# facebookresearch/seamless_communication

Hardware: AMD Instinct MI355X
Metric: S2ST utterances/sec (and real-time factor), seamlessM4T_v2_large, 10 s audio (higher is better)
Workload: dtype f32 activations x f16 weights, f32 accumulate

## Files before the change

### seamless_communication_amd/csrc/common.cpp

```cpp
#include "common.h"
#include <cstdlib>
#include <cstring>

namespace sc {

static thread_local char g_err[1024] = "";

void set_error(const char* fmt, ...) {
    va_list ap;
    va_start(ap, fmt);
    vsnprintf(g_err, sizeof(g_err), fmt, ap);
    va_end(ap);
}

const char* get_error() { return g_err; }

namespace knob {
namespace {
struct Knob {
    const char* name;
    int kind;
    const char* what;
};
const Knob knob_table[] = {
// ... 4 lines not shown
    {"SC_DECODER_GEN2", 1, "decoder step on the second-generation chain"},
    {"SC_VOC_SPLIT", 1, "vocoder ResBlock products on both fp16 planes of their activations again (bit 0 wide stages, bit 2 narrow stages); default: hi plane only"},
    {"SC_GEMM_GENERAL", 0, "general GEMM kernel instead of the fast path"}, {"SC_GEMM_PF2", 0, "GEMM prefetch depth"},
    {"SC_GEMM_GROUP_M", 0, "GEMM workgroup order"}, {"SC_GEMM_TILE", 0, "GEMM tile override"},
    {"SC_PS_TILE", 0, "DMA GEMM: largest tile"}, {"SC_PS_MIN256", 0, "DMA GEMM: tiles needed for 256 x 256"},
    {"SC_PS_MIN128", 0, "DMA GEMM: tiles needed for 128 x 128"},
    {"SC_PRESPLIT", 0, "0: Conformer operands split on the fly"}, {"SC_ENC_FUSE", 0, "0: separate Conformer element-wise launches"},
    {"SC_D3_RG_SMALL", 0, "decoder step: rows per row group, N = 1024 products"}, {"SC_D3_RG_FFN", 0, "decoder step: rows per row group, FFN-in"},
    {"SC_G3_STATIONARY", 0, "row-group products of wide steps: 0 one workgroup per row group, n = workgroup budget of the weight-stationary launch"},
    {"SC_G3_TILES", 0, "0: FFN-out of wide steps on the weight-stationary row-group walk instead of tile-owning waves"},
    {"SC_G3_TOUCH", 0, "weight-stationary products: bit 0 cooperative L2 touch of the activations, bit 1 K slices per XCD (FFN-out); default 3"},
    {"SC_D3_FFN_IN", 0, "decoder step: FFN-in workgroup shape"}, {"SC_D3_FFN_OUT", 0, "decoder step: FFN-out workgroup shape"},
    {"SC_T2U_GROUPS", 0, "NAR T2U: length buckets"}, {"SC_T2U_PACKED", 0, "0: NAR decoder on padded buckets"},
    {"SC_VOC_PS", 0, "0: vocoder wide stages on the register-staged convolution"}, {"SC_VOC_MRF", 0, "0: narrow vocoder stages as nine pair launches"},
    {"SC_VOC_GROUPS", 0, "vocoder: length buckets"}, {"SC_VOC_GROUP_OVERHEAD", 0, "vocoder: bucket planning overhead rows"},
    {"SC_VOC_STREAMS", 0, "vocoder: side chains"},
    {"SC_VOC_PACKED", 0, "0: ragged vocoder batches in length buckets on side chains instead of the packed pass"},
    {"SC_VOC_PACK_ROWS", 0, "vocoder: unit rows per packed group"},
    {"SC_ENGINE_RG_SMALL", 0, "decode engine: rows per row group, N = 1024 products"},
    {"SC_BEAM_COMPACT", 2, "0: beam search keeps finished utterances' slots"},
    {"SC_GREEDY_COMPACT", 2, "0: greedy generation keeps finished rows in their slots"}, {"SC_GREEDY_POLL", 2, "steps between looks at the finished flags"},
    {"SC_T2U_ENC_PACKED", 2, "0: T2U encoder over the padded rows on the fp32-operand GEMM"},
    {"SC_ENC_GLU_EPI", 2, "0: Conformer conv module writes both GLU halves and gates them in the depthwise kernel"},
};
constexpr int N_KNOBS = sizeof(knob_table) / sizeof(knob_table[0]);
struct State {
    bool set[N_KNOBS];
    int val[N_KNOBS];
    bool numerics = false;
};
const State& state() {
    static const State st = [] {
        State s{};
        const char* dn = getenv("SC_DEBUG_NUMERICS");
        s.numerics = dn && atoi(dn) != 0;
        for (int i = 0; i < N_KNOBS; ++i) {
            const char* e = getenv(knob_table[i].name);
            s.set[i] = e != nullptr && (knob_table[i].kind != 1 || s.numerics);
            s.val[i] = e ? atoi(e) : 0;
        }
        return s;
    }();
    return st;
}
int lookup(const char* name) {
    for (int i = 0; i < N_KNOBS; ++i)
// ... 43 lines not shown
```

### seamless_communication_amd/csrc/k_gemm.hip

```cpp
#include <atomic>
#include <cstdlib>

#include "device_util.h"

namespace sc {

std::atomic<int> g_force_general_gemm{0};

static constexpr int BK = 32;
static constexpr int LDS_LD = 40;

__device__ __forceinline__ float apply_in_act(float v, int in_act) {
    if (in_act == IN_LRELU_01) return v > 0.f ? v : 0.1f * v;
    if (in_act == IN_LRELU_001) return v > 0.f ? v : 0.01f * v;
    return v;
}

template <int BM, int BN, int WGM, int WGN, int AMODE, bool SPLIT>
__global__ __launch_bounds__(256) void gemm_kernel(GemmArgs p) {
    static_assert(WGM * WGN == 4, "4 waves per block");
    constexpr int WM = BM / WGM, WN = BN / WGN;
    constexpr int TM = WM / 32, TN = WN / 32;
    static_assert(TM >= 1 && TN >= 1, "wave tile must hold a 32x32 fragment");
    constexpr int A_IT = BM / 32;
    constexpr int B_IT = (BN * 4 + 255) / 256;

    __shared__ __attribute__((aligned(16))) _Float16 sAh[BM * LDS_LD];
    __shared__ __attribute__((aligned(16))) _Float16 sAl[SPLIT ? BM * LDS_LD : 8];
    __shared__ __attribute__((aligned(16))) _Float16 sB[BN * LDS_LD];

    const int tid = threadIdx.x;
    const int lane = tid & 63;
    const int wave = tid >> 6;
    const int wm = wave / WGN, wn = wave % WGN;
    const int m0 = blockIdx.y * BM;
    const int n0 = blockIdx.x * BN;
    const int phase = blockIdx.z;
    const __half* __restrict__ W = p.W + (int64_t)phase * p.w_phase_stride;
    const int out_off = p.out_off + phase * p.out_off_phase_step;

    const int a_kq = tid & 7;
// ... 131 lines not shown
#pragma unroll
            for (int i = 0; i < TM; ++i) {
                const int off = (wm * WM + i * 32 + frag_row) * LDS_LD + kb + frag_k;
                ah[i] = *reinterpret_cast<const half8_t*>(&sAh[off]);
                if (SPLIT) al[i] = *reinterpret_cast<const half8_t*>(&sAl[off]);
            }
#pragma unroll
            for (int j = 0; j < TN; ++j) {
                const int off = (wn * WN + j * 32 + frag_row) * LDS_LD + kb + frag_k;
                bf[j] = *reinterpret_cast<const half8_t*>(&sB[off]);
            }
#pragma unroll
            for (int i = 0; i < TM; ++i)
#pragma unroll
                for (int j = 0; j < TN; ++j) {
                    acc[i][j] = __builtin_amdgcn_mfma_f32_32x32x16_f16(ah[i], bf[j], acc[i][j], 0, 0, 0);
                    if (SPLIT)
                        acc[i][j] = __builtin_amdgcn_mfma_f32_32x32x16_f16(al[i], bf[j], acc[i][j], 0, 0, 0);
                }
        }
        __syncthreads();
    }

    const bool plain_rows = !p.item_off && (p.rows_per_batch == p.M) && p.out_mul == 1 && out_off == 0 && p.t_out == p.M;
    if (p.item_off && m0 + wm * WM + 4 * (lane >> 5) < p.M) cur.init(p, m0 + wm * WM + 4 * (lane >> 5));
#pragma unroll
    for (int i = 0; i < TM; ++i) {
#pragma unroll
        for (int r = 0; r < 16; ++r) {
            const int m = m0 + wm * WM + i * 32 + (r & 3) + 8 * (r >> 2) + 4 * (lane >> 5);
            if (m >= p.M) continue;
            int64_t row;
            if (plain_rows) {
                row = m;
            } else if (p.item_off) {
                cur.seek(p, m);
                const int dst_t = cur.q(m) * p.out_mul + out_off;
                if (dst_t < 0 || dst_t >= cur.t_out(p)) continue;
                row = cur.out_row0(p) + dst_t;
            } else {
                const int n = m / p.rows_per_batch;
                const int q = m - n * p.rows_per_batch;
                const int dst_t = q * p.out_mul + out_off;
                if (dst_t < 0 || dst_t >= p.t_out) continue;
                row = (int64_t)n * p.t_out + dst_t;
            }
#pragma unroll
            for (int j = 0; j < TN; ++j) {
                const int col = n0 + wn * WN + j * 32 + (lane & 31);
                if (col >= p.N) continue;
                float v = acc[i][j][r];
                if (p.bias) v += p.bias[col];
                v = act(v, p.act) * p.alpha;
                if (p.res) v += p.res[row * p.ldr + col];
                p.C[row * p.ldc + col] = v;
            }
        }
    }
}

template <int BM, int BN, int WGM, int WGN>
static void launch_cfg(const GemmArgs& a, hipStream_t s) {
    dim3 grid(cdiv(a.N, BN), cdiv(a.M, BM), a.phases);
    const bool vec_ok = (a.lda % 4 == 0) && ((reinterpret_cast<uintptr_t>(a.A) & 15) == 0);
    const int amode = (vec_ok && a.cin % 32 == 0) ? 1 : (vec_ok && a.cin % 4 == 0) ? 2 : 0;
    char name[64];
    snprintf(name, sizeof(name), "gemm_%dx%d_%s_%s", BM, BN, amode == 1 ? "vecA" : amode == 2 ? "vec4A" : "genA",
             a.split ? "split" : "f16");
    const double kreal = (double)a.taps * a.cin;
    const double flops = a.algo_flops > 0 ? a.algo_flops : 2.0 * a.M * a.N * kreal * a.phases;
    const double bytes = 4.0 * a.M * (double)a.cin * (a.stride < a.taps ? 1.0 : (double)a.taps) +
                         2.0 * a.N * (double)a.K * a.phases + 4.0 * a.M * (double)a.N * (a.res ? 2.0 : 1.0);
    prof::Scope scope(name, flops, bytes, s);
#define SC_GEMM_LAUNCH(AM, SP) hipLaunchKernelGGL((gemm_kernel<BM, BN, WGM, WGN, AM, SP>), grid, dim3(256), 0, s, a)
    if (a.split) {
        if (amode == 1) SC_GEMM_LAUNCH(1, true);
        else if (amode == 2) SC_GEMM_LAUNCH(2, true);
        else SC_GEMM_LAUNCH(0, true);
    } else {
        if (amode == 1) SC_GEMM_LAUNCH(1, false);
        else if (amode == 2) SC_GEMM_LAUNCH(2, false);
        else SC_GEMM_LAUNCH(0, false);
    }
#undef SC_GEMM_LAUNCH
}

void launch_gemm(const GemmArgs& a, hipStream_t s) {
    SC_CHECK(a.K % BK == 0, "gemm: K=%d must be a multiple of %d", a.K, BK);
    SC_CHECK(a.ldw % 8 == 0, "gemm: ldw=%lld must be a multiple of 8", (long long)a.ldw);
    SC_CHECK(a.M > 0 && a.N > 0, "gemm: empty problem M=%d N=%d", a.M, a.N);
    SC_CHECK(a.rows_per_batch > 0 && a.cin > 0, "gemm: rows_per_batch/cin unset");
    static const bool env_general = knob::is_set("SC_GEMM_GENERAL");
    SC_CHECK(a.act >= ACT_NONE && a.act <= ACT_GELU, "gemm: unknown activation %d", a.act);
    if (!env_general && !g_force_general_gemm.load(std::memory_order_relaxed) && gemm_fast_eligible(a)) {
        launch_gemm_fast(a, s);
        return;
    }
    const int64_t tiles128 = (int64_t)cdiv(a.M, 128) * cdiv(a.N, 128) * a.phases;
    if (a.M <= 32) {
        launch_cfg<32, 128, 1, 4>(a, s);
    } else if (a.N <= 32) {
        if ((int64_t)cdiv(a.M, 256) * a.phases >= 512) launch_cfg<256, 32, 4, 1>(a, s);
        else launch_cfg<128, 32, 4, 1>(a, s);
    } else if (a.N <= 64) {
        if ((int64_t)cdiv(a.M, 128) * a.phases >= 512) launch_cfg<128, 64, 2, 2>(a, s);
        else launch_cfg<64, 64, 2, 2>(a, s);
    } else if (tiles128 >= 256) {
        launch_cfg<128, 128, 2, 2>(a, s);
    } else {
        launch_cfg<64, 64, 2, 2>(a, s);
    }
    SC_LAUNCH_CHECK();
}

template <int MR>
__global__ __launch_bounds__(256) void gemv_kernel(const float* __restrict__ x, int64_t ldx,
// ... 76 lines not shown
```

### seamless_communication_amd/csrc/k_gemm2.hip

```cpp
#include <algorithm>
#include <cstdlib>

#include "device_util.h"

namespace sc {

namespace {

constexpr int GEMM_GROUP_M_DEFAULT = 1;
constexpr int GEMM_PF2_DEFAULT = 1;
constexpr int FBK = 32;
constexpr int FLD = 40;

template <int TM, int TN, int WM, int WN, int ACT, bool HAS_RES>
__device__ __forceinline__ void epilogue(const GemmArgs& p, float16_t (&acc)[TM][TN], int m0w, int n0w, int lane,
                                         int out_off, bool plain_rows) {
    float bcol[TN];
    int col[TN];
#pragma unroll
    for (int j = 0; j < TN; ++j) {
        col[j] = n0w + j * 32 + (lane & 31);
        bcol[j] = (p.bias && col[j] < p.N) ? p.bias[col[j]] : 0.f;
    }
    GemmItemCursor cur;
    if (p.item_off && m0w + 4 * (lane >> 5) < p.M) cur.init(p, m0w + 4 * (lane >> 5));
#pragma unroll
    for (int i = 0; i < TM; ++i) {
#pragma unroll
        for (int r = 0; r < 16; ++r) {
            const int m = m0w + i * 32 + (r & 3) + 8 * (r >> 2) + 4 * (lane >> 5);
            if (m >= p.M) continue;
            int64_t row;
            if (plain_rows) {
                row = m;
            } else if (p.item_off) {
                cur.seek(p, m);
                const int dst_t = cur.q(m) * p.out_mul + out_off;
                if (dst_t < 0 || dst_t >= cur.t_out(p)) continue;
                row = cur.out_row0(p) + dst_t;
            } else {
                const int n = m / p.rows_per_batch;
                const int q = m - n * p.rows_per_batch;
                const int dst_t = q * p.out_mul + out_off;
                if (dst_t < 0 || dst_t >= p.t_out) continue;
                row = (int64_t)n * p.t_out + dst_t;
            }
#pragma unroll
            for (int j = 0; j < TN; ++j) {
                if (col[j] >= p.N) continue;
                float v = act<ACT>(acc[i][j][r] + bcol[j]) * p.alpha;
                if (HAS_RES) v += p.res[row * p.ldr + col[j]];
                p.C[row * p.ldc + col[j]] = v;
            }
        }
    }
}

template <int TM, int TN, int WN, int EP_LD, int ACT, bool HAS_RES>
__device__ __forceinline__ void epilogue_lds(const GemmArgs& p, float16_t (&acc)[TM][TN], float* ep, int m0w, int n0w, int lane,
                                             int out_off, bool plain_rows) {
    constexpr int LPR = WN / 4;
    constexpr int RPG = 16 / LPR;
    constexpr int RPI = 4 * RPG;
    const int l5 = lane & 31;
    const bool g1 = (l5 >= 4 && l5 < 12) || (l5 >= 16 && l5 < 20) || l5 >= 28;
    const int rank = g1 ? (l5 < 12 ? l5 - 4 : l5 < 20 ? l5 - 8 : l5 - 16) : (l5 < 4 ? l5 : l5 < 16 ? l5 - 8 : l5 - 12);
    const int grp = (lane >> 5) * 2 + (g1 ? 1 : 0);
    const int row_in = grp * RPG + rank / LPR;
    const int c0 = (rank % LPR) * 4;
    const int col = n0w + c0;
    const bool vec_ok = (col + 3 < p.N) && (p.ldc % 4 == 0) && (!HAS_RES || p.ldr % 4 == 0) &&
                        ((reinterpret_cast<uintptr_t>(p.C) | (HAS_RES ? reinterpret_cast<uintptr_t>(p.res) : 0)) & 15) == 0;
    f32x4_t b4 = {0.f, 0.f, 0.f, 0.f};
    if (p.bias) {
#pragma unroll
        for (int e = 0; e < 4; ++e) b4[e] = (col + e < p.N) ? p.bias[col + e] : 0.f;
    }
    GemmItemCursor cur;
    if (p.item_off && m0w + row_in < p.M) cur.init(p, m0w + row_in);
#pragma unroll
    for (int i = 0; i < TM; ++i) {
#pragma unroll
        for (int j = 0; j < TN; ++j)
#pragma unroll
            for (int r = 0; r < 16; ++r) ep[((r & 3) + 8 * (r >> 2) + 4 * (lane >> 5)) * EP_LD + j * 32 + (lane & 31)] = acc[i][j][r];
#pragma unroll
        for (int it = 0; it < 32 / RPI; ++it) {
            const int rr = it * RPI + row_in;
            const int m = m0w + i * 32 + rr;
            const f32x4_t a = *reinterpret_cast<const f32x4_t*>(ep + rr * EP_LD + c0);
            if (m >= p.M || col >= p.N) continue;
            int64_t row;
            if (plain_rows) {
                row = m;
            } else if (p.item_off) {
                cur.seek(p, m);
                const int dst_t = cur.q(m) * p.out_mul + out_off;
                if (dst_t < 0 || dst_t >= cur.t_out(p)) continue;
                row = cur.out_row0(p) + dst_t;
            } else {
                const int n = m / p.rows_per_batch;
                const int q = m - n * p.rows_per_batch;
                const int dst_t = q * p.out_mul + out_off;
                if (dst_t < 0 || dst_t >= p.t_out) continue;
                row = (int64_t)n * p.t_out + dst_t;
            }
            f32x4_t v;
#pragma unroll
            for (int e = 0; e < 4; ++e) v[e] = act<ACT>(a[e] + b4[e]) * p.alpha;
            if (vec_ok) {
                if (HAS_RES) v += *reinterpret_cast<const f32x4_t*>(p.res + row * p.ldr + col);
                *reinterpret_cast<f32x4_t*>(p.C + row * p.ldc + col) = v;
            } else {
#pragma unroll
                for (int e = 0; e < 4; ++e) {
                    if (col + e >= p.N) continue;
                    float x = v[e];
                    if (HAS_RES) x += p.res[row * p.ldr + col + e];
                    p.C[row * p.ldc + col + e] = x;
                }
            }
        }
    }
}

template <int BM, int BN, int WGM, int WGN, bool IN_ACT, bool CONV>
__global__ __launch_bounds__(256) void gemm_fast_kernel(GemmArgs p, int tiles_n, int tiles_mn, int tiles_total,
                                                        int tiles_per_xcd, float in_slope, int group_m) {
    static_assert(WGM * WGN == 4, "4 waves per block");
    constexpr int WM = BM / WGM, WN = BN / WGN;
    constexpr int TM = WM / 32, TN = WN / 32;
    static_assert(TM >= 1 && TN >= 1, "wave tile must hold a 32x32 fragment");
    constexpr int A_IT = BM / 32;
    constexpr int B_IT = (BN * 4 + 255) / 256;

    __shared__ __attribute__((aligned(16))) _Float16 sAh[2][BM * FLD];
    __shared__ __attribute__((aligned(16))) _Float16 sAl[2][BM * FLD];
    __shared__ __attribute__((aligned(16))) _Float16 sB[2][BN * FLD];

    const int bid = blockIdx.x;
    const int tile = (bid & 7) * tiles_per_xcd + (bid >> 3);
    if (tile >= tiles_total) return;
    const int phase = tile / tiles_mn;
    const int rem = tile - phase * tiles_mn;
    int tm, tn;
    {
        const int per_group = group_m * tiles_n;
        const int g = rem / per_group;
        const int in_g = rem - g * per_group;
// ... 131 lines not shown
    SC_STORE_SLAB(0);
    __syncthreads();
    for (int s = 0; s + 1 < nslab; ++s) {
        const int st = s & 1;
        if (++cs == slabs_per_tap) {
            cs = 0;
            set_tap(++tap);
        }
        SC_LOAD_SLAB(cs * FBK, (s + 1) * FBK);
        __builtin_amdgcn_sched_barrier(0);
        SC_COMPUTE_SLAB(st);
        __builtin_amdgcn_sched_barrier(0);
        SC_STORE_SLAB(st ^ 1);
        __syncthreads();
    }
    {
        const int st = (nslab - 1) & 1;
        SC_COMPUTE_SLAB(st);
    }
#undef SC_LOAD_SLAB
#undef SC_STORE_SLAB
#undef SC_COMPUTE_SLAB

    const bool plain_rows = !p.item_off && (p.rows_per_batch == p.M) && p.out_mul == 1 && out_off == 0 && p.t_out == p.M;
    const int m0w = m0 + wm * WM, n0w = n0 + wn * WN;
#define SC_EPI(ACT)                                                                               \
    do {                                                                                          \
        if (p.res) epilogue<TM, TN, WM, WN, ACT, true>(p, acc, m0w, n0w, lane, out_off, plain_rows); \
        else epilogue<TM, TN, WM, WN, ACT, false>(p, acc, m0w, n0w, lane, out_off, plain_rows);    \
    } while (0)
    if (p.act == ACT_NONE) SC_EPI(ACT_NONE);
    else if (p.act == ACT_RELU) SC_EPI(ACT_RELU);
    else if (p.act == ACT_SILU) SC_EPI(ACT_SILU);
    else if (p.act == ACT_TANH) SC_EPI(ACT_TANH);
    else SC_EPI(ACT_GELU);
#undef SC_EPI
}

template <int BM, int BN, int WGM, int WGN, bool IN_ACT>
__global__ __launch_bounds__(256) void gemm_fast2_kernel(GemmArgs p, int tiles_n, int tiles_mn, int tiles_total,
                                                         int tiles_per_xcd, float in_slope, uint32_t a_bytes, uint32_t w_bytes) {
    static_assert(WGM * WGN == 4, "4 waves per block");
    constexpr int WM = BM / WGM, WN = BN / WGN;
    constexpr int TM = WM / 32, TN = WN / 32;
    constexpr int A_IT = BM / 32;
    constexpr int B_IT = (BN * 4 + 255) / 256;

    constexpr int EP_LD = WN + 4;
    static_assert(4 * 32 * EP_LD * 4 <= (4 * BM + 2 * BN) * FLD * 2, "epilogue tiles must fit in the stage memory");
    __shared__ __attribute__((aligned(16))) _Float16 smem_all[(4 * BM + 2 * BN) * FLD];
    _Float16(*sAh)[BM * FLD] = reinterpret_cast<_Float16(*)[BM * FLD]>(smem_all);
    _Float16(*sAl)[BM * FLD] = reinterpret_cast<_Float16(*)[BM * FLD]>(smem_all + 2 * BM * FLD);
    _Float16(*sB)[BN * FLD] = reinterpret_cast<_Float16(*)[BN * FLD]>(smem_all + 4 * BM * FLD);

    const int bid = blockIdx.x;
    const int tile = (bid & 7) * tiles_per_xcd + (bid >> 3);
    if (tile >= tiles_total) return;
    const int phase = tile / tiles_mn;
    const int rem = tile - phase * tiles_mn;
    const int tm = rem / tiles_n;
    const int tn = rem - tm * tiles_n;

// ... 132 lines not shown
        __builtin_amdgcn_sched_barrier(0);                                        \
        SC2_COMPUTE((S) & 1);                                                     \
        __builtin_amdgcn_sched_barrier(0);                                        \
        if ((S) + 1 < nslab) SC2_STORE(ANEXT, BNEXT, ((S) + 1) & 1);              \
        __syncthreads();                                                          \
    } while (0)

    set_tap(0);
    SC2_LOAD(a_reg0, b_reg0, 0, 0, 0u);
    SC2_STORE(a_reg0, b_reg0, 0);
    SC2_ADVANCE();
    SC2_LOAD(a_reg1, b_reg1, cs * (FBK * 4), FBK * 2, 0u);
    __syncthreads();
    for (int s = 0; s < nslab; s += 2) {
        SC2_STEP(s, a_reg0, b_reg0, a_reg1, b_reg1);
        SC2_STEP(s + 1, a_reg1, b_reg1, a_reg0, b_reg0);
    }
#undef SC2_STEP
#undef SC2_ADVANCE
#undef SC2_LOAD
#undef SC2_STORE
#undef SC2_COMPUTE

    const bool plain_rows = !p.item_off && (p.rows_per_batch == p.M) && p.out_mul == 1 && out_off == 0 && p.t_out == p.M;
    const int m0w = m0 + wm * WM, n0w = n0 + wn * WN;
    float* ep = reinterpret_cast<float*>(smem_all) + wave * (32 * EP_LD);
#define SC_EPI(ACT)                                                                                             \
    do {                                                                                                        \
        if (p.res) epilogue_lds<TM, TN, WN, EP_LD, ACT, true>(p, acc, ep, m0w, n0w, lane, out_off, plain_rows);  \
        else epilogue_lds<TM, TN, WN, EP_LD, ACT, false>(p, acc, ep, m0w, n0w, lane, out_off, plain_rows);       \
    } while (0)
    if (p.act == ACT_NONE) SC_EPI(ACT_NONE);
    else if (p.act == ACT_RELU) SC_EPI(ACT_RELU);
    else if (p.act == ACT_SILU) SC_EPI(ACT_SILU);
    else if (p.act == ACT_TANH) SC_EPI(ACT_TANH);
    else SC_EPI(ACT_GELU);
#undef SC_EPI
}

template <int BM, int BN, int WGM, int WGN>
void launch_fast_cfg(const GemmArgs& a, hipStream_t s) {
    const int tiles_m = cdiv(a.M, BM), tiles_n = cdiv(a.N, BN);
    const int tiles_mn = tiles_m * tiles_n;
    const int64_t total64 = (int64_t)tiles_mn * a.phases;
    SC_CHECK(total64 < (1ll << 30), "gemm: %lld tiles", (long long)total64);
    const int tiles_total = (int)total64;
    const int tiles_per_xcd = cdiv(tiles_total, 8);
    char name[64];
    snprintf(name, sizeof(name), "gemm_%dx%d_fast_split", BM, BN);
    const double kreal = (double)a.taps * a.cin;
    const double flops = a.algo_flops > 0 ? a.algo_flops : 2.0 * a.M * a.N * kreal * a.phases;
    const double bytes = 4.0 * a.M * (double)a.cin * (a.stride < a.taps ? 1.0 : (double)a.taps) +
                         2.0 * a.N * (double)a.K * a.phases + 4.0 * a.M * (double)a.N * (a.res ? 2.0 : 1.0);
    prof::Scope scope(name, flops, bytes, s);
    const dim3 grid(tiles_per_xcd * 8);
    static const int env_pf2 = knob::value("SC_GEMM_PF2", GEMM_PF2_DEFAULT);
    const int64_t a_bytes64 = (a.item_off ? (int64_t)a.M - (int64_t)a.n_items * a.item_extra : (int64_t)(a.M / a.rows_per_batch) * a.t_in) * a.lda * 4;
    const int64_t w_bytes64 = (int64_t)a.N * a.ldw * 2;
    if (env_pf2 && a.K % (2 * FBK) == 0 && (a.item_off || a.M % a.rows_per_batch == 0) && a_bytes64 < (1ll << 31) && w_bytes64 < (1ll << 31)) {
        const float slope = a.in_act == IN_LRELU_01 ? 0.1f : a.in_act == IN_LRELU_001 ? 0.01f : 0.f;
        if (a.in_act == IN_NONE)
            hipLaunchKernelGGL((gemm_fast2_kernel<BM, BN, WGM, WGN, false>), grid, dim3(256), 0, s, a, tiles_n, tiles_mn,
                               tiles_total, tiles_per_xcd, slope, (uint32_t)a_bytes64, (uint32_t)w_bytes64);
        else
            hipLaunchKernelGGL((gemm_fast2_kernel<BM, BN, WGM, WGN, true>), grid, dim3(256), 0, s, a, tiles_n, tiles_mn,
                               tiles_total, tiles_per_xcd, slope, (uint32_t)a_bytes64, (uint32_t)w_bytes64);
        return;
    }
    static const int env_gm = knob::value("SC_GEMM_GROUP_M", 0);
    const int group_m = std::max(1, std::min(env_gm > 0 ? env_gm : GEMM_GROUP_M_DEFAULT, tiles_m));
    const bool conv = a.taps != 1 || a.stride != 1 || a.pad != 0 || a.in_lens != nullptr;
    if (a.in_act == IN_NONE) {
        if (conv)
            hipLaunchKernelGGL((gemm_fast_kernel<BM, BN, WGM, WGN, false, true>), grid, dim3(256), 0, s, a, tiles_n,
                               tiles_mn, tiles_total, tiles_per_xcd, 0.f, group_m);
        else
            hipLaunchKernelGGL((gemm_fast_kernel<BM, BN, WGM, WGN, false, false>), grid, dim3(256), 0, s, a, tiles_n,
                               tiles_mn, tiles_total, tiles_per_xcd, 0.f, group_m);
    } else {
        const float slope = a.in_act == IN_LRELU_01 ? 0.1f : 0.01f;
        hipLaunchKernelGGL((gemm_fast_kernel<BM, BN, WGM, WGN, true, true>), grid, dim3(256), 0, s, a, tiles_n, tiles_mn,
                           tiles_total, tiles_per_xcd, slope, group_m);
    }
}

}

bool gemm_fast_eligible(const GemmArgs& a) {
    return a.split == 1 && a.cin % FBK == 0 && a.K == a.taps * a.cin && a.lda % 4 == 0 &&
           (reinterpret_cast<uintptr_t>(a.A) & 15) == 0 && a.ldw % 8 == 0 && a.M > 32 &&
           a.N > 32 &&
           (a.in_act == IN_NONE || a.in_act == IN_LRELU_01 || a.in_act == IN_LRELU_001);
}

void launch_gemm_fast(const GemmArgs& a, hipStream_t s) {
// ... 21 lines not shown
```

### seamless_communication_amd/csrc/k_misc.hip

```cpp
#include "device_util.h"

namespace sc {

__global__ __launch_bounds__(256) void embed_tokens_kernel(const int* __restrict__ tokens, int rows,
                                                           const __half* __restrict__ emb, int M,
                                                           float scale, const float* __restrict__ pos_table,
                                                           const int* __restrict__ d_pos, int t_per_batch,
                                                           float* __restrict__ out, int64_t ldo) {
    const int row = blockIdx.x;
    const int tok = tokens[row];
    const int pos = (d_pos ? *d_pos : 0) + (t_per_batch > 0 ? row % t_per_batch : 0);
    const __half* e = emb + (int64_t)tok * M;
    const float* pe = pos_table + (int64_t)pos * M;
    for (int c = threadIdx.x; c < M; c += 256) out[(int64_t)row * ldo + c] = __half2float(e[c]) * scale + pe[c];
}

void launch_embed_tokens(const int* tokens, int rows, const __half* emb, int M, float scale,
                         const float* pos_table, const int* d_pos, int t_per_batch, float* out, int64_t ldo,
                         hipStream_t s) {
    if (rows <= 0) return;
    hipLaunchKernelGGL(embed_tokens_kernel, dim3(rows), dim3(256), 0, s, tokens, rows, emb, M, scale, pos_table,
                       d_pos, t_per_batch, out, ldo);
    SC_LAUNCH_CHECK();
}
// ... 356 lines not shown
    for (int o = 32; o > 0; o >>= 1) acc += __shfl_xor(acc, o);
    if (lane == 0) {
        const int n = row / t_per_batch, t = row - n * t_per_batch;
        int d = 0;
        if (!lens || t < lens[n]) {
            const float x = acc + b[0];
            const float r = rintf((expf(x) - 1.0f) * duration_factor);
            long long dl = r >= 1000000.f ? 1000000 : (long long)r;
            if (dl < (long long)min_dur) dl = min_dur;
            if (dl > 1000000) dl = 1000000;
            d = (int)dl;
        }
        durations[row] = d;
    }
}
void launch_durations(const float* h, int64_t ld, const float* w, const float* b, int rows, int H, int t_per_batch,
                      const int* lens, float duration_factor, int min_dur, int* durations, hipStream_t s) {
    if (rows <= 0) return;
    hipLaunchKernelGGL(durations_kernel, dim3(cdiv(rows, 4)), dim3(256), 0, s, h, ld, w, b, rows, H, t_per_batch, lens,
                       duration_factor, min_dur, durations);
    SC_LAUNCH_CHECK();
}

__global__ __launch_bounds__(256) void vocoder_embed_kernel(const int* __restrict__ units, int T,
                                                            const __half* __restrict__ dict, int E,
                                                            const __half* __restrict__ lang, int Lg,
                                                            const int* __restrict__ lang_idx,
                                                            const __half* __restrict__ spkr, int Sp,
                                                            const int* __restrict__ spkr_idx,
                                                            float* __restrict__ out, const int* __restrict__ item_off, int n_items) {
    const int row = blockIdx.x;
    const int n = item_off ? item_search(n_items, row, [&](int i) { return item_off[i]; }) : row / T;
    const int C = Lg + E + Sp;
    const __half* l = lang + (int64_t)lang_idx[n] * Lg;
    const __half* d = dict + (int64_t)units[row] * E;
    const __half* sp = spkr + (int64_t)spkr_idx[n] * Sp;
    float* o = out + (int64_t)row * C;
    for (int c = threadIdx.x; c < C; c += 256) {
        __half v;
        if (c < Lg) v = l[c];
        else if (c < Lg + E) v = d[c - Lg];
        else v = sp[c - Lg - E];
        o[c] = __half2float(v);
    }
}
void launch_vocoder_embed(const int* units, int nb, int T, const __half* dict, int E, const __half* lang, int Lg,
                          const int* lang_idx, const __half* spkr, int Sp, const int* spkr_idx, float* out,
                          hipStream_t s, const int* item_off, int rows_total) {
    const int rows = item_off ? rows_total : nb * T;
    if (rows <= 0) return;
    hipLaunchKernelGGL(vocoder_embed_kernel, dim3(rows), dim3(256), 0, s, units, T, dict, E, lang, Lg, lang_idx, spkr,
                       Sp, spkr_idx, out, item_off, nb);
    SC_LAUNCH_CHECK();
}

__global__ void avg3_kernel(const float* __restrict__ a, const float* __restrict__ b, const float* __restrict__ c,
                            float* __restrict__ out, int64_t n) {
    for (int64_t i = (int64_t)blockIdx.x * blockDim.x + threadIdx.x; i < n; i += (int64_t)gridDim.x * blockDim.x)
        out[i] = ((a[i] + b[i]) + c[i]) / 3.0f;
}
__global__ void split_f32_kernel(const float* __restrict__ x, __half* __restrict__ hi, __half* __restrict__ lo, int64_t n4) {
    for (int64_t i = (int64_t)blockIdx.x * blockDim.x + threadIdx.x; i < n4; i += (int64_t)gridDim.x * blockDim.x) {
        const f32x4_t v = reinterpret_cast<const f32x4_t*>(x)[i];
        const half4_t h = __builtin_convertvector(v, half4_t);
        reinterpret_cast<half4_t*>(hi)[i] = h;
        reinterpret_cast<half4_t*>(lo)[i] = __builtin_convertvector(v - __builtin_convertvector(h, f32x4_t), half4_t);
    }
}
void launch_split_f32(const float* x, __half* hi, __half* lo, int64_t n, hipStream_t s) {
    SC_CHECK(n % 4 == 0, "split_f32: n must be a multiple of 4");
    if (n <= 0) return;
    hipLaunchKernelGGL(split_f32_kernel, dim3(grid_for(n / 4)), dim3(256), 0, s, x, hi, lo, n / 4);
    SC_LAUNCH_CHECK();
}
// ... 217 lines not shown
```

### seamless_communication_amd/csrc/kernels.h

```cpp
#pragma once
#include <atomic>
#include <vector>

#include "common.h"
#include "boost_list.h"
#include "prof.h"

struct sc_tsm_opts;

namespace sc {

enum Act { ACT_NONE = 0, ACT_RELU = 1, ACT_SILU = 2, ACT_TANH = 3, ACT_GELU = 4 };
enum InAct { IN_NONE = 0, IN_LRELU_01 = 1, IN_LRELU_001 = 2 };

__device__ __forceinline__ int argmax_stored_index(int idx) { return idx == 0x7fffffff ? 0 : idx; }

__device__ __forceinline__ float lrelu_in(float x, float slope) {
    const float r = fmaxf(x, 0.f) + slope * fminf(x, 0.f);
    return x != x ? x : r;
}

struct GemmArgs {
    const float* A = nullptr;
    int64_t lda = 0;
    const __half* W = nullptr;
    int64_t ldw = 0;
    int64_t w_phase_stride = 0;
    const float* bias = nullptr;
    const float* res = nullptr;
    int64_t ldr = 0;
    float* C = nullptr;
    int64_t ldc = 0;
    int M = 0;
    int N = 0;
    int K = 0;
    int rows_per_batch = 0;
    int t_in = 0;
    int t_out = 0;
    int taps = 1, cin = 0, dil = 0, stride = 1, pad = 0;
    int out_mul = 1, out_off = 0, out_off_phase_step = 0;
    const int* in_lens = nullptr;
    int in_act = IN_NONE;
    int act = ACT_NONE;
    float alpha = 1.0f;
    int phases = 1;
    int split = 1;
    double algo_flops = 0;
    const int* item_off = nullptr;
    int n_items = 0, item_mul = 1, item_extra = 0, item_out_mul = 1;
};

#if defined(__HIPCC__)
template <typename F>
__device__ __forceinline__ int item_search(int n, int key, F first) {
    int lo = 0, hi = n - 1;
    while (lo < hi) {
        const int mid = (lo + hi + 1) >> 1;
        if (first(mid) <= key) lo = mid;
        else hi = mid - 1;
    }
    return lo;
}

struct GemmItemCursor {
    int n = 0, start = 0, next = 0x7fffffff;
    __device__ __forceinline__ static int first(const GemmArgs& p, int i) { return p.item_off[i] * p.item_mul + i * p.item_extra; }
    __device__ __forceinline__ void init(const GemmArgs& p, int m) {
        n = item_search(p.n_items, m, [&](int i) { return first(p, i); });
// ... 543 lines not shown
    const float* w = nullptr;
    const float* b = nullptr;
    int H = 0;
    float* e = nullptr;
    int s_char = 0;
    const int* lens = nullptr;
    const int* target = nullptr;
    const float* lo = nullptr;
    const float* hi = nullptr;
    int min_dur = 1;
    int* durations = nullptr;
    float* factor = nullptr;
    long long* total = nullptr;
    int* flags = nullptr;
};
void launch_fit_durations(const FitArgs& a, int n, hipStream_t s);
void check_fit_items(const char* who, int n, const int32_t* h_target, const float* h_lo, const float* h_hi);
void run_time_stretch(const char* who, const float* d_in, int n, int64_t in_stride, const int64_t* h_in_len, const int64_t* h_out_len,
                      const ::sc_tsm_opts* opts, bool with_out, float* d_out, int64_t out_stride, int32_t* h_centres, int64_t m_stride);
void launch_vocoder_embed(const int* units, int nb, int T, const __half* dict, int E,
                          const __half* lang, int Lg, const int* lang_idx, const __half* spkr, int Sp,
                          const int* spkr_idx, float* out , hipStream_t s,
                          const int* item_off = nullptr , int rows_total = 0);
void launch_avg3(const float* a, const float* b, const float* c, float* out, int64_t n, hipStream_t s);
bool conv_to_mono_supported(int cin, int cout, int k, int stride, int pad, int dil, int act);
void launch_conv_to_mono(const float* x, const __half* w_packed, const float* bias, int nb, int T, int cin, int k, float in_slope, int act,
                         float* y, hipStream_t s, const int* item_off = nullptr ,
                         int item_mul = 1, int64_t rows_total = 0);
void launch_item_row_pos(const int* item_off, int n_items, int mul, int rows, int2* row_pos, hipStream_t s);
void launch_scatter_items(const float* src, const int* item_off, const int* item_of, int n_items, int mul, int longest, int64_t dst_stride,
                          float* dst, hipStream_t s);
void launch_fill_i32(int* p, int v, int n, hipStream_t s);
void launch_add_i32(int* p, int v, hipStream_t s);

constexpr int ROWSWAP_MAX_LAYERS = 32;
constexpr int ROWSWAP_MAX_PAIRS = 64;
struct RowSwapArgs {
    float* k[ROWSWAP_MAX_LAYERS];
    float* v[ROWSWAP_MAX_LAYERS];
    float* cross[ROWSWAP_MAX_LAYERS];
    int layers = 0, pairs = 0;
    unsigned char src[ROWSWAP_MAX_PAIRS], dst[ROWSWAP_MAX_PAIRS];
    int M = 0, cap = 0, s_enc = 0, filled = 0;
    int* tok = nullptr;
    int* finished = nullptr;
    int* out_len = nullptr;
// ... 250 lines not shown
```

### seamless_communication_amd/csrc/model_load.hip

```cpp
#include <cmath>
#include <cstdio>
#include <cstring>

#include <cstdlib>

#include "loader.h"

namespace sc {

DevicePool::~DevicePool() { release_all(); }

static int debug_fill_byte() {
    static const int v = [] {
        (void)knob::is_set("SC_DEBUG_FILL");
        const char* e = getenv("SC_DEBUG_FILL");
        return e && *e ? (int)strtol(e, nullptr, 0) & 0xff : -1;
    }();
    return v;
}

void* DevicePool::debug_filled(void* p, size_t bytes) {
    const int v = debug_fill_byte();
    if (v >= 0 && p && stream_) {
        hipStreamCaptureStatus st = hipStreamCaptureStatusNone;
// ... 845 lines not shown
    a.K = c.kpad;
    a.t_in = t_in;
    a.t_out = t_in * c.stride;
    a.taps = c.taps;
    a.cin = c.cin;
    a.dil = -1;
    a.stride = 1;
    a.pad = 0;
    a.out_mul = c.stride;
    a.out_off = -c.pad;
    a.out_off_phase_step = 1;
    a.phases = c.stride;
    a.in_act = in_act;
    a.algo_flops = 2.0 * nb * (double)t_in * c.cin * c.cout * c.k;
    if (pk) {
        a.M = pk->rows() * mul + pk->n;
        a.item_off = pk->d_off;
        a.n_items = pk->n;
        a.item_mul = mul;
        a.item_extra = 1;
        a.item_out_mul = c.stride;
        a.algo_flops = 2.0 * pk->rows() * (double)mul * c.cin * c.cout * c.k;
    }
    launch_gemm(a, m.stream);
}

}
```

### seamless_communication_amd/csrc/model_t2u.hip

```cpp
#include <cstdlib>

#include "model.h"

namespace sc {

namespace {

void text_to_char_seqs(const Model& m, const int32_t* text_seqs, int n, int s_text, std::vector<int32_t>& char_lens,
                       std::vector<std::vector<int32_t>>& char_ids) {
    const sc_config& c = m.cfg;
    SC_CHECK(!m.tok_len.empty(), "sc_t2u_nar: sc_set_nar_tables() has not been called");
    char_lens.assign((size_t)n * s_text, 0);
    char_ids.assign(n, {});
    const int S = s_text - 2;
    for (int b = 0; b < n; ++b) {
        std::vector<int32_t> toks;
        for (int i = 0; i < S; ++i) {
            int32_t t = text_seqs[(size_t)b * s_text + 2 + i];
            if (t == c.eos_idx) t = c.pad_idx;
            SC_CHECK(t >= 0 && t < (int)m.tok_len.size(), "sc_t2u_nar: token id %d out of range", t);
            toks.push_back(t);
        }
        int nsub = 0;
        for (int32_t t : toks) nsub += (t != c.pad_idx);
// ... 479 lines not shown
        const std::vector<int32_t>& gids = keep_alive[3 * g + 2];
        const int Lg = (int)(gids.size() / grp.size());
        for (size_t gi = 0; gi < grp.size(); ++gi)
            for (int t = 0; t < ulens[grp[gi]]; ++t) ids[(size_t)grp[gi] * Su + t] = gids[gi * Lg + t];
    }
    launches = 0;
    finish(ids, rows_done);
}

namespace {

void vocode_batch(Model& m, const int* d_units, const int* d_lang, const int* d_spkr, int n, int T, float* d_wav,
                  const PackedItems* pk = nullptr, const float* d_rows_in = nullptr, int post_act = ACT_TANH, int plane_split = -1) {
    const sc_config& c = m.cfg;
    const int E = c.voc_embedding_dim, Lg = c.voc_lang_embedding_dim, Sp = c.voc_spkr_embedding_dim;
    int ch = c.voc_upsample_initial_channel;
    int t = T;
    int rate = 1;
    const size_t rows0 = pk ? (size_t)pk->rows() : (size_t)n * T;
    Buf<float> x;
    if (d_rows_in) {
        x = Buf<float>(m.pp(), rows0 * ch);
        conv1d(m, d_rows_in, m.voc_pre, nullptr, x, n, T, 1, 3, 1, nullptr, IN_NONE, ACT_NONE, pk, 1);
    } else {
        Buf<float> in(m.pp(), rows0 * (E + Lg + Sp));
        launch_vocoder_embed(d_units, n, T, m.voc_dict, E, m.voc_lang, Lg, d_lang, m.voc_spkr, Sp, d_spkr, in, m.stream, pk ? pk->d_off : nullptr,
                             (int)rows0);
        x = Buf<float>(m.pp(), rows0 * ch);
        conv1d(m, in, m.voc_pre, nullptr, x, n, T, 1, 3, 1, nullptr, IN_NONE, ACT_NONE, pk, 1);
    }
    const int nk = c.voc_num_resblock_kernels;
    SC_CHECK(nk == 3, "sc_vocode: %d resblock kernels (only 3 is implemented)", nk);
    static const int voc_split_knob = knob::value("SC_VOC_SPLIT", 0);
    const int voc_split = plane_split >= 0 ? plane_split : voc_split_knob;
    const int voc_single = (voc_split & 1 ? 0 : 1) | (voc_split & 4 ? 0 : 4);
    for (int i = 0; i < c.voc_num_upsamples; ++i) {
        const ConvT& up = m.voc_ups[i];
        const int t2 = t * up.stride;
        const int rate2 = rate * up.stride;
        ch = up.cout;
        const size_t rows = rows0 * rate2;
        const size_t sz = rows * ch;
        Buf<float> y(m.pp(), sz), tmp, ra, rb, rout[3];
        const auto need = [&](Buf<float>& b) -> float* {
            if (!b.get()) b = Buf<float>(m.pp(), sz);
            return b.get();
// ... 448 lines not shown
```

Baseline: 341.7.

## Merge transposed-conv phases into one grouped GEMM; run vocoder conv_pre on fp16 plane

Vocoder transposed convolutions now run as a single product whose N spans all stride phases, with a grouped epilogue that scatters each column group to its phase's output rows, instead of separate tile sets per phase. Separately, the vocoder embedding is gathered directly into an fp16 plane and conv_pre runs on the presplit DMA GEMM rather than on fp32 rows split on the fly. Both are meant to cut launch and tile overhead and operand conversion traffic. In exchange they add template variants, a heavier scattered epilogue and alignment preconditions. The fp16 plane also drops the lo plane of an input that is already exact fp16, so results should not change.

```diff
diff --git a/seamless_communication_amd/csrc/common.cpp b/seamless_communication_amd/csrc/common.cpp
--- a/seamless_communication_amd/csrc/common.cpp
+++ b/seamless_communication_amd/csrc/common.cpp
@@ -50,6 +50,8 @@
     {"SC_GREEDY_COMPACT", 2, "0: greedy generation keeps finished rows in their slots"}, {"SC_GREEDY_POLL", 2, "steps between looks at the finished flags"},
     {"SC_T2U_ENC_PACKED", 2, "0: T2U encoder over the padded rows on the fp32-operand GEMM"},
     {"SC_ENC_GLU_EPI", 2, "0: Conformer conv module writes both GLU halves and gates them in the depthwise kernel"},
+    {"SC_VOC_CT_MERGED", 2, "0: transposed convolutions as one set of tiles per phase instead of one product over all phases"},
+    {"SC_VOC_PRE_PLANE", 2, "0: vocoder conv_pre on fp32 rows split on the fly instead of the gathered fp16 plane on the DMA GEMM"},
 };
 constexpr int N_KNOBS = sizeof(knob_table) / sizeof(knob_table[0]);
 struct State {
diff --git a/seamless_communication_amd/csrc/k_gemm.hip b/seamless_communication_amd/csrc/k_gemm.hip
--- a/seamless_communication_amd/csrc/k_gemm.hip
+++ b/seamless_communication_amd/csrc/k_gemm.hip
@@ -16,7 +16,7 @@
     return v;
 }
 
-template <int BM, int BN, int WGM, int WGN, int AMODE, bool SPLIT>
+template <int BM, int BN, int WGM, int WGN, int AMODE, bool SPLIT, bool GROUPED = false>
 __global__ __launch_bounds__(256) void gemm_kernel(GemmArgs p) {
     static_assert(WGM * WGN == 4, "4 waves per block");
     constexpr int WM = BM / WGM, WN = BN / WGN;
@@ -194,8 +194,18 @@
         __syncthreads();
     }
 
-    const bool plain_rows = !p.item_off && (p.rows_per_batch == p.M) && p.out_mul == 1 && out_off == 0 && p.t_out == p.M;
+    const bool plain_rows = !GROUPED && !p.item_off && (p.rows_per_batch == p.M) && p.out_mul == 1 && out_off == 0 && p.t_out == p.M;
     if (p.item_off && m0 + wm * WM + 4 * (lane >> 5) < p.M) cur.init(p, m0 + wm * WM + 4 * (lane >> 5));
+    int g_off[TN], g_col[TN];
+    if (GROUPED) {
+#pragma unroll
+        for (int j = 0; j < TN; ++j) {
+            const int col = n0 + wn * WN + j * 32 + (lane & 31);
+            const int g = col / p.col_group;
+            g_off[j] = g * p.out_off_phase_step;
+            g_col[j] = col - g * p.col_group;
+        }
+    }
 #pragma unroll
     for (int i = 0; i < TM; ++i) {
 #pragma unroll
@@ -203,25 +213,43 @@
             const int m = m0 + wm * WM + i * 32 + (r & 3) + 8 * (r >> 2) + 4 * (lane >> 5);
             if (m >= p.M) continue;
             int64_t row;
+            int dst_t0 = 0, t_out = 0;
             if (plain_rows) {
                 row = m;
             } else if (p.item_off) {
                 cur.seek(p, m);
                 const int dst_t = cur.q(m) * p.out_mul + out_off;
-                if (dst_t < 0 || dst_t >= cur.t_out(p)) continue;
-                row = cur.out_row0(p) + dst_t;
+                if (GROUPED) {
+                    dst_t0 = dst_t, t_out = cur.t_out(p);
+                    row = cur.out_row0(p);
+                } else {
+                    if (dst_t < 0 || dst_t >= cur.t_out(p)) continue;
+                    row = cur.out_row0(p) + dst_t;
+                }
             } else {
                 const int n = m / p.rows_per_batch;
                 const int q = m - n * p.rows_per_batch;
                 const int dst_t = q * p.out_mul + out_off;
-                if (dst_t < 0 || dst_t >= p.t_out) continue;
-                row = (int64_t)n * p.t_out + dst_t;
+                if (GROUPED) {
+                    dst_t0 = dst_t, t_out = p.t_out;
+                    row = (int64_t)n * p.t_out;
+                } else {
+                    if (dst_t < 0 || dst_t >= p.t_out) continue;
+                    row = (int64_t)n * p.t_out + dst_t;
+                }
             }
 #pragma unroll
             for (int j = 0; j < TN; ++j) {
                 const int col = n0 + wn * WN + j * 32 + (lane & 31);
                 if (col >= p.N) continue;
                 float v = acc[i][j][r];
+                if (GROUPED) {
+                    const int dst_t = dst_t0 + g_off[j];
+                    if (dst_t < 0 || dst_t >= t_out) continue;
+                    if (p.bias) v += p.bias[g_col[j]];
+                    p.C[(row + dst_t) * p.ldc + g_col[j]] = act(v, p.act) * p.alpha;
+                    continue;
+                }
                 if (p.bias) v += p.bias[col];
                 v = act(v, p.act) * p.alpha;
                 if (p.res) v += p.res[row * p.ldr + col];
@@ -245,7 +273,10 @@
                          2.0 * a.N * (double)a.K * a.phases + 4.0 * a.M * (double)a.N * (a.res ? 2.0 : 1.0);
     prof::Scope scope(name, flops, bytes, s);
 #define SC_GEMM_LAUNCH(AM, SP) hipLaunchKernelGGL((gemm_kernel<BM, BN, WGM, WGN, AM, SP>), grid, dim3(256), 0, s, a)
-    if (a.split) {
+    if (a.col_group) {
+        SC_CHECK(amode == 1 && a.split, "gemm: column groups need cin %% 32 == 0, 16-byte aligned rows and the split product");
+        hipLaunchKernelGGL((gemm_kernel<BM, BN, WGM, WGN, 1, true, true>), grid, dim3(256), 0, s, a);
+    } else if (a.split) {
         if (amode == 1) SC_GEMM_LAUNCH(1, true);
         else if (amode == 2) SC_GEMM_LAUNCH(2, true);
         else SC_GEMM_LAUNCH(0, true);
@@ -264,6 +295,9 @@
     SC_CHECK(a.rows_per_batch > 0 && a.cin > 0, "gemm: rows_per_batch/cin unset");
     static const bool env_general = knob::is_set("SC_GEMM_GENERAL");
     SC_CHECK(a.act >= ACT_NONE && a.act <= ACT_GELU, "gemm: unknown activation %d", a.act);
+    SC_CHECK(a.col_group == 0 || (a.col_group % 4 == 0 && a.N % a.col_group == 0 && a.phases == 1 && !a.res && a.act == ACT_NONE && a.ldc % 4 == 0 &&
+                                  (reinterpret_cast<uintptr_t>(a.C) & 15) == 0),
+             "gemm: column groups of %d in N=%d (phases %d): no residual / activation, 16-byte aligned output rows", a.col_group, a.N, a.phases);
     if (!env_general && !g_force_general_gemm.load(std::memory_order_relaxed) && gemm_fast_eligible(a)) {
         launch_gemm_fast(a, s);
         return;
diff --git a/seamless_communication_amd/csrc/k_gemm2.hip b/seamless_communication_amd/csrc/k_gemm2.hip
--- a/seamless_communication_amd/csrc/k_gemm2.hip
+++ b/seamless_communication_amd/csrc/k_gemm2.hip
@@ -12,7 +12,21 @@
 constexpr int FBK = 32;
 constexpr int FLD = 40;
 
-template <int TM, int TN, int WM, int WN, int ACT, bool HAS_RES>
+struct GroupedRow {
+    int64_t row0;
+    int dst_t0, t_out;
+};
+__device__ __forceinline__ GroupedRow grouped_row(const GemmArgs& p, GemmItemCursor& cur, int m, int out_off) {
+    if (p.item_off) {
+        cur.seek(p, m);
+        return {cur.out_row0(p), cur.q(m) * p.out_mul + out_off, cur.t_out(p)};
+    }
+    const int n = m / p.rows_per_batch;
+    const int q = m - n * p.rows_per_batch;
+    return {(int64_t)n * p.t_out, q * p.out_mul + out_off, p.t_out};
+}
+
+template <int TM, int TN, int WM, int WN, int ACT, bool HAS_RES, bool GROUPED = false>
 __device__ __forceinline__ void epilogue(const GemmArgs& p, float16_t (&acc)[TM][TN], int m0w, int n0w, int lane,
                                          int out_off, bool plain_rows) {
     float bcol[TN];
@@ -20,10 +34,36 @@
 #pragma unroll
     for (int j = 0; j < TN; ++j) {
         col[j] = n0w + j * 32 + (lane & 31);
-        bcol[j] = (p.bias && col[j] < p.N) ? p.bias[col[j]] : 0.f;
+        bcol[j] = (!GROUPED && p.bias && col[j] < p.N) ? p.bias[col[j]] : 0.f;
     }
     GemmItemCursor cur;
     if (p.item_off && m0w + 4 * (lane >> 5) < p.M) cur.init(p, m0w + 4 * (lane >> 5));
+    if (GROUPED) {
+        int g_off[TN], g_col[TN];
+#pragma unroll
+        for (int j = 0; j < TN; ++j) {
+            const int g = col[j] / p.col_group;
+            g_off[j] = g * p.out_off_phase_step;
+            g_col[j] = col[j] - g * p.col_group;
+            bcol[j] = (p.bias && col[j] < p.N) ? p.bias[g_col[j]] : 0.f;
+        }
+#pragma unroll
+        for (int i = 0; i < TM; ++i) {
+#pragma unroll
+            for (int r = 0; r < 16; ++r) {
+                const int m = m0w + i * 32 + (r & 3) + 8 * (r >> 2) + 4 * (lane >> 5);
+                if (m >= p.M) continue;
+                const GroupedRow gr = grouped_row(p, cur, m, out_off);
+#pragma unroll
+                for (int j = 0; j < TN; ++j) {
+                    const int dst_t = gr.dst_t0 + g_off[j];
+                    if (col[j] >= p.N || dst_t < 0 || dst_t >= gr.t_out) continue;
+                    p.C[(gr.row0 + dst_t) * p.ldc + g_col[j]] = act<ACT>(acc[i][j][r] + bcol[j]) * p.alpha;
+                }
+            }
+        }
+        return;
+    }
 #pragma unroll
     for (int i = 0; i < TM; ++i) {
 #pragma unroll
@@ -56,7 +96,7 @@
     }
 }
 
-template <int TM, int TN, int WN, int EP_LD, int ACT, bool HAS_RES>
+template <int TM, int TN, int WN, int EP_LD, int ACT, bool HAS_RES, bool GROUPED = false>
 __device__ __forceinline__ void epilogue_lds(const GemmArgs& p, float16_t (&acc)[TM][TN], float* ep, int m0w, int n0w, int lane,
                                              int out_off, bool plain_rows) {
     constexpr int LPR = WN / 4;
@@ -71,10 +111,13 @@
     const int col = n0w + c0;
     const bool vec_ok = (col + 3 < p.N) && (p.ldc % 4 == 0) && (!HAS_RES || p.ldr % 4 == 0) &&
                         ((reinterpret_cast<uintptr_t>(p.C) | (HAS_RES ? reinterpret_cast<uintptr_t>(p.res) : 0)) & 15) == 0;
+    const int grp_c = GROUPED ? col / p.col_group : 0;
+    const int g_off = grp_c * p.out_off_phase_step;
+    const int dcol = col - grp_c * p.col_group;
     f32x4_t b4 = {0.f, 0.f, 0.f, 0.f};
     if (p.bias) {
 #pragma unroll
-        for (int e = 0; e < 4; ++e) b4[e] = (col + e < p.N) ? p.bias[col + e] : 0.f;
+        for (int e = 0; e < 4; ++e) b4[e] = (col + e < p.N) ? p.bias[dcol + e] : 0.f;
     }
     GemmItemCursor cur;
     if (p.item_off && m0w + row_in < p.M) cur.init(p, m0w + row_in);
@@ -91,7 +134,12 @@
             const f32x4_t a = *reinterpret_cast<const f32x4_t*>(ep + rr * EP_LD + c0);
             if (m >= p.M || col >= p.N) continue;
             int64_t row;
-            if (plain_rows) {
+            if (GROUPED) {
+                const GroupedRow gr = grouped_row(p, cur, m, out_off);
+                const int dst_t = gr.dst_t0 + g_off;
+                if (dst_t < 0 || dst_t >= gr.t_out) continue;
+                row = gr.row0 + dst_t;
+            } else if (plain_rows) {
                 row = m;
             } else if (p.item_off) {
                 cur.seek(p, m);
@@ -109,22 +157,22 @@
 #pragma unroll
             for (int e = 0; e < 4; ++e) v[e] = act<ACT>(a[e] + b4[e]) * p.alpha;
             if (vec_ok) {
-                if (HAS_RES) v += *reinterpret_cast<const f32x4_t*>(p.res + row * p.ldr + col);
-                *reinterpret_cast<f32x4_t*>(p.C + row * p.ldc + col) = v;
+                if (HAS_RES) v += *reinterpret_cast<const f32x4_t*>(p.res + row * p.ldr + dcol);
+                *reinterpret_cast<f32x4_t*>(p.C + row * p.ldc + dcol) = v;
             } else {
 #pragma unroll
                 for (int e = 0; e < 4; ++e) {
                     if (col + e >= p.N) continue;
                     float x = v[e];
-                    if (HAS_RES) x += p.res[row * p.ldr + col + e];
-                    p.C[row * p.ldc + col + e] = x;
+                    if (HAS_RES) x += p.res[row * p.ldr + dcol + e];
+                    p.C[row * p.ldc + dcol + e] = x;
                 }
             }
         }
     }
 }
 
-template <int BM, int BN, int WGM, int WGN, bool IN_ACT, bool CONV>
+template <int BM, int BN, int WGM, int WGN, bool IN_ACT, bool CONV, bool GROUPED = false>
 __global__ __launch_bounds__(256) void gemm_fast_kernel(GemmArgs p, int tiles_n, int tiles_mn, int tiles_total,
                                                         int tiles_per_xcd, float in_slope, int group_m) {
     static_assert(WGM * WGN == 4, "4 waves per block");
@@ -302,13 +350,17 @@
 #undef SC_STORE_SLAB
 #undef SC_COMPUTE_SLAB
 
-    const bool plain_rows = !p.item_off && (p.rows_per_batch == p.M) && p.out_mul == 1 && out_off == 0 && p.t_out == p.M;
+    const bool plain_rows = !GROUPED && !p.item_off && (p.rows_per_batch == p.M) && p.out_mul == 1 && out_off == 0 && p.t_out == p.M;
     const int m0w = m0 + wm * WM, n0w = n0 + wn * WN;
 #define SC_EPI(ACT)                                                                               \
     do {                                                                                          \
         if (p.res) epilogue<TM, TN, WM, WN, ACT, true>(p, acc, m0w, n0w, lane, out_off, plain_rows); \
         else epilogue<TM, TN, WM, WN, ACT, false>(p, acc, m0w, n0w, lane, out_off, plain_rows);    \
     } while (0)
+    if (GROUPED) {
+        epilogue<TM, TN, WM, WN, ACT_NONE, false, true>(p, acc, m0w, n0w, lane, out_off, false);
+        return;
+    }
     if (p.act == ACT_NONE) SC_EPI(ACT_NONE);
     else if (p.act == ACT_RELU) SC_EPI(ACT_RELU);
     else if (p.act == ACT_SILU) SC_EPI(ACT_SILU);
@@ -317,7 +369,7 @@
 #undef SC_EPI
 }
 
-template <int BM, int BN, int WGM, int WGN, bool IN_ACT>
+template <int BM, int BN, int WGM, int WGN, bool IN_ACT, bool GROUPED = false>
 __global__ __launch_bounds__(256) void gemm_fast2_kernel(GemmArgs p, int tiles_n, int tiles_mn, int tiles_total,
                                                          int tiles_per_xcd, float in_slope, uint32_t a_bytes, uint32_t w_bytes) {
     static_assert(WGM * WGN == 4, "4 waves per block");
@@ -496,7 +548,7 @@
 #undef SC2_STORE
 #undef SC2_COMPUTE
 
-    const bool plain_rows = !p.item_off && (p.rows_per_batch == p.M) && p.out_mul == 1 && out_off == 0 && p.t_out == p.M;
+    const bool plain_rows = !GROUPED && !p.item_off && (p.rows_per_batch == p.M) && p.out_mul == 1 && out_off == 0 && p.t_out == p.M;
     const int m0w = m0 + wm * WM, n0w = n0 + wn * WN;
     float* ep = reinterpret_cast<float*>(smem_all) + wave * (32 * EP_LD);
 #define SC_EPI(ACT)                                                                                             \
@@ -504,6 +556,10 @@
         if (p.res) epilogue_lds<TM, TN, WN, EP_LD, ACT, true>(p, acc, ep, m0w, n0w, lane, out_off, plain_rows);  \
         else epilogue_lds<TM, TN, WN, EP_LD, ACT, false>(p, acc, ep, m0w, n0w, lane, out_off, plain_rows);       \
     } while (0)
+    if (GROUPED) {
+        epilogue_lds<TM, TN, WN, EP_LD, ACT_NONE, false, true>(p, acc, ep, m0w, n0w, lane, out_off, false);
+        return;
+    }
     if (p.act == ACT_NONE) SC_EPI(ACT_NONE);
     else if (p.act == ACT_RELU) SC_EPI(ACT_RELU);
     else if (p.act == ACT_SILU) SC_EPI(ACT_SILU);
@@ -533,7 +589,13 @@
     const int64_t w_bytes64 = (int64_t)a.N * a.ldw * 2;
     if (env_pf2 && a.K % (2 * FBK) == 0 && (a.item_off || a.M % a.rows_per_batch == 0) && a_bytes64 < (1ll << 31) && w_bytes64 < (1ll << 31)) {
         const float slope = a.in_act == IN_LRELU_01 ? 0.1f : a.in_act == IN_LRELU_001 ? 0.01f : 0.f;
-        if (a.in_act == IN_NONE)
+        if (a.col_group && a.in_act == IN_NONE)
+            hipLaunchKernelGGL((gemm_fast2_kernel<BM, BN, WGM, WGN, false, true>), grid, dim3(256), 0, s, a, tiles_n, tiles_mn,
+                               tiles_total, tiles_per_xcd, slope, (uint32_t)a_bytes64, (uint32_t)w_bytes64);
+        else if (a.col_group)
+            hipLaunchKernelGGL((gemm_fast2_kernel<BM, BN, WGM, WGN, true, true>), grid, dim3(256), 0, s, a, tiles_n, tiles_mn,
+                               tiles_total, tiles_per_xcd, slope, (uint32_t)a_bytes64, (uint32_t)w_bytes64);
+        else if (a.in_act == IN_NONE)
             hipLaunchKernelGGL((gemm_fast2_kernel<BM, BN, WGM, WGN, false>), grid, dim3(256), 0, s, a, tiles_n, tiles_mn,
                                tiles_total, tiles_per_xcd, slope, (uint32_t)a_bytes64, (uint32_t)w_bytes64);
         else
@@ -544,7 +606,15 @@
     static const int env_gm = knob::value("SC_GEMM_GROUP_M", 0);
     const int group_m = std::max(1, std::min(env_gm > 0 ? env_gm : GEMM_GROUP_M_DEFAULT, tiles_m));
     const bool conv = a.taps != 1 || a.stride != 1 || a.pad != 0 || a.in_lens != nullptr;
-    if (a.in_act == IN_NONE) {
+    if (a.col_group) {
+        const float slope = a.in_act == IN_LRELU_01 ? 0.1f : a.in_act == IN_LRELU_001 ? 0.01f : 0.f;
+        if (a.in_act == IN_NONE)
+            hipLaunchKernelGGL((gemm_fast_kernel<BM, BN, WGM, WGN, false, true, true>), grid, dim3(256), 0, s, a, tiles_n,
+                               tiles_mn, tiles_total, tiles_per_xcd, slope, group_m);
+        else
+            hipLaunchKernelGGL((gemm_fast_kernel<BM, BN, WGM, WGN, true, true, true>), grid, dim3(256), 0, s, a, tiles_n,
+                               tiles_mn, tiles_total, tiles_per_xcd, slope, group_m);
+    } else if (a.in_act == IN_NONE) {
         if (conv)
             hipLaunchKernelGGL((gemm_fast_kernel<BM, BN, WGM, WGN, false, true>), grid, dim3(256), 0, s, a, tiles_n,
                                tiles_mn, tiles_total, tiles_per_xcd, 0.f, group_m);
diff --git a/seamless_communication_amd/csrc/k_misc.hip b/seamless_communication_amd/csrc/k_misc.hip
--- a/seamless_communication_amd/csrc/k_misc.hip
+++ b/seamless_communication_amd/csrc/k_misc.hip
@@ -1,3 +1,5 @@
+#include <type_traits>
+
 #include "device_util.h"
 
 namespace sc {
@@ -402,26 +404,28 @@
     SC_LAUNCH_CHECK();
 }
 
+template <typename OUT>
 __global__ __launch_bounds__(256) void vocoder_embed_kernel(const int* __restrict__ units, int T,
                                                             const __half* __restrict__ dict, int E,
                                                             const __half* __restrict__ lang, int Lg,
                                                             const int* __restrict__ lang_idx,
                                                             const __half* __restrict__ spkr, int Sp,
                                                             const int* __restrict__ spkr_idx,
-                                                            float* __restrict__ out, const int* __restrict__ item_off, int n_items) {
+                                                            OUT* __restrict__ out, const int* __restrict__ item_off, int n_items) {
     const int row = blockIdx.x;
     const int n = item_off ? item_search(n_items, row, [&](int i) { return item_off[i]; }) : row / T;
     const int C = Lg + E + Sp;
     const __half* l = lang + (int64_t)lang_idx[n] * Lg;
     const __half* d = dict + (int64_t)units[row] * E;
     const __half* sp = spkr + (int64_t)spkr_idx[n] * Sp;
-    float* o = out + (int64_t)row * C;
+    OUT* o = out + (int64_t)row * C;
     for (int c = threadIdx.x; c < C; c += 256) {
         __half v;
         if (c < Lg) v = l[c];
         else if (c < Lg + E) v = d[c - Lg];
         else v = sp[c - Lg - E];
-        o[c] = __half2float(v);
+        if constexpr (std::is_same<OUT, __half>::value) o[c] = v;
+        else o[c] = __half2float(v);
     }
 }
 void launch_vocoder_embed(const int* units, int nb, int T, const __half* dict, int E, const __half* lang, int Lg,
@@ -429,7 +433,16 @@
                           hipStream_t s, const int* item_off, int rows_total) {
     const int rows = item_off ? rows_total : nb * T;
     if (rows <= 0) return;
-    hipLaunchKernelGGL(vocoder_embed_kernel, dim3(rows), dim3(256), 0, s, units, T, dict, E, lang, Lg, lang_idx, spkr,
+    hipLaunchKernelGGL(vocoder_embed_kernel<float>, dim3(rows), dim3(256), 0, s, units, T, dict, E, lang, Lg, lang_idx, spkr,
+                       Sp, spkr_idx, out, item_off, nb);
+    SC_LAUNCH_CHECK();
+}
+void launch_vocoder_embed_plane(const int* units, int nb, int T, const __half* dict, int E, const __half* lang, int Lg,
+                                const int* lang_idx, const __half* spkr, int Sp, const int* spkr_idx, __half* out,
+                                hipStream_t s, const int* item_off, int rows_total) {
+    const int rows = item_off ? rows_total : nb * T;
+    if (rows <= 0) return;
+    hipLaunchKernelGGL(vocoder_embed_kernel<__half>, dim3(rows), dim3(256), 0, s, units, T, dict, E, lang, Lg, lang_idx, spkr,
                        Sp, spkr_idx, out, item_off, nb);
     SC_LAUNCH_CHECK();
 }
diff --git a/seamless_communication_amd/csrc/kernels.h b/seamless_communication_amd/csrc/kernels.h
--- a/seamless_communication_amd/csrc/kernels.h
+++ b/seamless_communication_amd/csrc/kernels.h
@@ -44,6 +44,7 @@
     int act = ACT_NONE;
     float alpha = 1.0f;
     int phases = 1;
+    int col_group = 0;
     int split = 1;
     double algo_flops = 0;
     const int* item_off = nullptr;
@@ -633,6 +634,9 @@
                           const __half* lang, int Lg, const int* lang_idx, const __half* spkr, int Sp,
                           const int* spkr_idx, float* out , hipStream_t s,
                           const int* item_off = nullptr , int rows_total = 0);
+void launch_vocoder_embed_plane(const int* units, int nb, int T, const __half* dict, int E, const __half* lang, int Lg,
+                                const int* lang_idx, const __half* spkr, int Sp, const int* spkr_idx, __half* out, hipStream_t s,
+                                const int* item_off = nullptr, int rows_total = 0);
 void launch_avg3(const float* a, const float* b, const float* c, float* out, int64_t n, hipStream_t s);
 bool conv_to_mono_supported(int cin, int cout, int k, int stride, int pad, int dil, int act);
 void launch_conv_to_mono(const float* x, const __half* w_packed, const float* bias, int nb, int T, int cin, int k, float in_slope, int act,
diff --git a/seamless_communication_amd/csrc/model_load.hip b/seamless_communication_amd/csrc/model_load.hip
--- a/seamless_communication_amd/csrc/model_load.hip
+++ b/seamless_communication_amd/csrc/model_load.hip
@@ -891,6 +891,13 @@
         a.item_out_mul = c.stride;
         a.algo_flops = 2.0 * pk->rows() * (double)mul * c.cin * c.cout * c.k;
     }
+    if (knob::live("SC_VOC_CT_MERGED", 1) != 0 && c.stride > 1 && c.cin % 32 == 0 && c.cout % 4 == 0 && c.kpad == c.taps * c.cin &&
+        ((reinterpret_cast<uintptr_t>(x) | reinterpret_cast<uintptr_t>(y)) & 15) == 0) {
+        a.N = c.stride * c.cout;
+        a.col_group = c.cout;
+        a.phases = 1;
+        a.w_phase_stride = 0;
+    }
     launch_gemm(a, m.stream);
 }
 
diff --git a/seamless_communication_amd/csrc/model_t2u.hip b/seamless_communication_amd/csrc/model_t2u.hip
--- a/seamless_communication_amd/csrc/model_t2u.hip
+++ b/seamless_communication_amd/csrc/model_t2u.hip
@@ -525,6 +525,19 @@
     if (d_rows_in) {
         x = Buf<float>(m.pp(), rows0 * ch);
         conv1d(m, d_rows_in, m.voc_pre, nullptr, x, n, T, 1, 3, 1, nullptr, IN_NONE, ACT_NONE, pk, 1);
+    } else if (const int C0 = E + Lg + Sp; knob::live("SC_VOC_PRE_PLANE", 1) != 0 && g_force_general_gemm.load(std::memory_order_relaxed) == 0 &&
+                                           rows0 > 0 && C0 % 32 == 0 && m.voc_pre.cin == C0 && m.voc_pre.kpad == C0 * m.voc_pre.k && m.voc_pre.k == 7 &&
+                                           m.voc_pre.cout % 4 == 0 && (int64_t)rows0 * C0 * 2 < (1ll << 31)) {
+        Buf<__half> in(m.pp(), rows0 * C0);
+        launch_vocoder_embed_plane(d_units, n, T, m.voc_dict, E, m.voc_lang, Lg, d_lang, m.voc_spkr, Sp, d_spkr, in, m.stream, pk ? pk->d_off : nullptr,
+                                   (int)rows0);
+        Buf<int2> row_pos;
+        if (pk) {
+            row_pos = Buf<int2>(m.pp(), rows0);
+            launch_item_row_pos(pk->d_off, pk->n, 1, (int)rows0, row_pos.get(), m.stream);
+        }
+        x = Buf<float>(m.pp(), rows0 * ch);
+        conv1d_presplit(m, in, nullptr, m.voc_pre, nullptr, x, nullptr, nullptr, n, T, 3, 1, nullptr, ACT_NONE, (int)rows0, row_pos.get(), 1.0f, 0);
     } else {
         Buf<float> in(m.pp(), rows0 * (E + Lg + Sp));
         launch_vocoder_embed(d_units, n, T, m.voc_dict, E, m.voc_lang, Lg, d_lang, m.voc_spkr, Sp, d_spkr, in, m.stream, pk ? pk->d_off : nullptr,
```

Result: no change. 344.8, median of 6 (+0.9%).
